# qasimyu/simuscop

Measured on AMD Instinct MI355X. Metric: simulated paired reads/sec (whole node) at 30x WGS PE150, higher is better.
Workload: dtype u32

## Files before the change

simuscop_amd/csrc/sg_kernels.hip:

```cpp
#include <algorithm>
#include <cstdlib>
#include <type_traits>

#include "sg_device.h"

namespace sg {

template <int ROUNDS>
__device__ __forceinline__ void philox4x32(uint32_t c0, uint32_t c1, uint32_t c2, uint32_t c3,
                                           uint32_t k0, uint32_t k1, uint32_t out[4]) {
  const uint32_t M0 = 0xD2511F53u, M1 = 0xCD9E8D57u;
#pragma unroll
  for (int r = 0; r < ROUNDS; r++) {
    const uint64_t p0 = (uint64_t)M0 * c0, p1 = (uint64_t)M1 * c2;
    const uint32_t hi0 = (uint32_t)(p0 >> 32), lo0 = (uint32_t)p0;
    const uint32_t hi1 = (uint32_t)(p1 >> 32), lo1 = (uint32_t)p1;
    c0 = __builtin_amdgcn_bitop3_b32(hi1, c1, k0, 0x96);
    c1 = lo1;
    c2 = __builtin_amdgcn_bitop3_b32(hi0, c3, k1, 0x96);
    c3 = lo0;
    k0 += 0x9E3779B9u;
    k1 += 0xBB67AE85u;
  }
  out[0] = c0; out[1] = c1; out[2] = c2; out[3] = c3;
// ... 22 lines not shown
  philox4x32_10(slot + B.slot_offset, j, f >> 2, dev_ctx(KIND_AUX, mate, B.batch_id), B.k0, B.k1, x);
  uint32_t l = f & 3;
  return l == 0 ? x[0] : l == 1 ? x[1] : l == 2 ? x[2] : x[3];
}

__device__ __forceinline__ uint32_t ndigits(uint32_t v) {
  return v < 10 ? 1 : v < 100 ? 2 : v < 1000 ? 3 : v < 10000 ? 4 : v < 100000 ? 5 : v < 1000000 ? 6
       : v < 10000000 ? 7 : v < 100000000 ? 8 : v < 1000000000 ? 9 : 10;
}

#define PLAN_S 16

__device__ __forceinline__ bool plan_attempt(const DevProfile& P, const DevBatch& B, const sg_window& win, uint64_t w,
                                             uint32_t attempt, uint64_t clen, uint32_t c3, PairRec& r, const uint32_t* isz_row,
                                             uint32_t seg_size, uint64_t chain_off) {
  uint32_t x[4];
  philox4x32_10((uint32_t)w + B.win_offset, attempt, 0, c3, B.k0, B.k1, x);
  const double frac = __dmul_rn((double)x[0], 1.0 / 4294967296.0);
  const double v = __dadd_rn((double)win.spos, __dmul_rn((double)win.len, frac));
  const uint32_t pos = (uint32_t)(long long)v;
  uint32_t isz;
  if (B.paired) isz = isz_row ? (uint32_t)P.isz_min + row_search(isz_row, P.isz_lg, x[1]) : (uint32_t)P.fixed_isz;
  else isz = win.len;
  const uint64_t avail = clen - (win.hap_base + pos);
  const uint32_t flen = avail < (uint64_t)isz ? (uint32_t)avail : isz;
  const uint32_t strand = B.paired ? 0u : (x[2] >> 31);
  r.win = (uint32_t)w; r.fl = flen | (strand << 31);
  r.namepos = pos % seg_size;
  r.foff = chain_off + win.hap_base + pos;
  r.pad = 0;
  return flen >= (uint32_t)P.L;
}

__global__ __launch_bounds__(256) void plan_kernel(DevProfile P, DevBatch B) {
  __shared__ uint32_t isz_lds[1025];
  const uint32_t* isz_row = P.isz_row;
  if (P.isz_row && P.isz_lg <= 10u) {
    for (uint32_t i = threadIdx.x; i < (1u << P.isz_lg) + 1u; i += blockDim.x) isz_lds[i] = P.isz_row[i];
    isz_row = isz_lds;
  }
  __syncthreads();
  if (blockIdx.x == 0)
    for (uint32_t i = threadIdx.x; i < kTotalsBytes / 4u; i += blockDim.x) ((uint32_t*)B.totals)[i] = 0u;
  const uint64_t gid = (uint64_t)blockIdx.x * blockDim.x + threadIdx.x;
  const uint64_t w = gid / PLAN_S;
  const uint32_t j = (uint32_t)(gid % PLAN_S);
  if (w >= B.n_windows) return;
  const sg_window win = B.windows[w];
  const int n = win.n_reads;
  const uint32_t planned = n <= 0 ? 0u : (B.paired ? ((uint32_t)n + 1u) / 2u : (uint32_t)n);
  const uint64_t clen = B.chain_len[win.chain];
  const uint32_t seg_size = B.seg_size[win.seg];
  const uint64_t chain_off = B.chain_off[win.chain];
  const uint32_t c3 = dev_ctx(KIND_PLAN, 0, B.batch_id);
  const uint64_t last_start = win.hap_base + win.spos + win.len - 1u;
  const uint64_t need = B.paired ? (uint64_t)P.isz_hi : (uint64_t)win.len;
  const uint32_t shortest = B.paired ? (uint32_t)P.isz_lo : win.len;
  const bool safe = last_start + need <= clen && shortest >= (uint32_t)P.L;
  if (safe) {
    for (uint32_t k = j; k < planned; k += PLAN_S) {
      PairRec r;
      plan_attempt(P, B, win, w, k, clen, c3, r, isz_row, seg_size, chain_off);
      r.k = k;
      B.pairs[win.slot_base + k] = r;
    }
    if (j == 0) B.win_actual[w] = planned;
    return;
  }
  if (j != 0) return;
  uint32_t done = 0, fail = 0, attempt = 0;
  while (done < planned) {
    PairRec r;
    if (!plan_attempt(P, B, win, w, attempt++, clen, c3, r, isz_row, seg_size, chain_off)) {
      if (++fail > 1000) break;
      continue;
    }
    r.k = done;
    B.pairs[win.slot_base + done] = r;
    done++;
  }
  for (uint32_t k = done; k < planned; k++) {
    PairRec r;
    r.win = (uint32_t)w; r.namepos = 0; r.fl = 0; r.k = k; r.foff = 0; r.pad = 0;
    B.pairs[win.slot_base + k] = r;
  }
  B.win_actual[w] = done;
}

__global__ __launch_bounds__(64) void namebase_kernel(DevBatch B) {
  const uint32_t s = blockIdx.x;
  const uint32_t lane = threadIdx.x;
  const uint32_t w0 = B.seg_first_window[s], w1 = B.seg_first_window[s + 1];
  uint32_t carry = 0;
  for (uint32_t base = w0; base < w1; base += 64) {
    uint32_t w = base + lane;
    uint32_t v = w < w1 ? B.win_actual[w] : 0u;
    uint32_t incl = v;
#pragma unroll
    for (int d = 1; d < 64; d <<= 1) {
      uint32_t t = __shfl_up(incl, d);
      if ((int)lane >= d) incl += t;
    }
    if (w < w1) B.win_namebase[w] = carry + incl - v;
    carry += __shfl(incl, 63);
  }
  if (lane == 0) atomicAdd((unsigned long long*)&B.totals[2], (unsigned long long)carry);
}

__device__ __forceinline__ void wave_lds_sync() {
  __builtin_amdgcn_fence(__ATOMIC_RELEASE, "wavefront");
  __builtin_amdgcn_wave_barrier();
  __builtin_amdgcn_fence(__ATOMIC_ACQUIRE, "wavefront");
}

__device__ __forceinline__ uint64_t rec_offset(const DevBatch& B, uint32_t m, uint32_t t) {
  const uint32_t blk = t >> 8;
  const uint64_t* segbase = (const uint64_t*)((const uint8_t*)B.totals + kTotalsSegBase);
  return segbase[m * 16u + (blk >> B.seg_shift)] + B.blkbase[(size_t)m * ((B.n_slots + 255u) >> 8) + blk] +
         B.recloc[(size_t)m * B.n_slots + t];
}

__global__ __launch_bounds__(256) void indel_kernel(DevProfile P, DevBatch B) {
  __shared__ uint4 row_lds[256 * 3];
  __shared__ uint16_t cand[512];
  __shared__ uint32_t cand_n;
  __shared__ uint2 found[2][256];
  __shared__ uint32_t found_first[2][256];
  __shared__ uint32_t wave_len[2][4];
  const uint32_t tid = threadIdx.x, lane = tid & 63u, wv = tid >> 6;
  const uint32_t t = blockIdx.x * blockDim.x + tid;
  const uint32_t nm = B.paired ? 2u : 1u;
  uint4* const wave_rows = row_lds + (tid & ~63u) * 3u;
  uint4* const my_row = wave_rows + lane * 3u;
  const uint32_t t_wave = t - lane;
  __shared__ uint64_t gap_lds[256];
  const uint64_t* gap = P.gap_row;
  if ((uint32_t)P.L + 1u <= 256u) {
    for (uint32_t i = tid; i <= (uint32_t)P.L; i += blockDim.x) gap_lds[i] = P.gap_row[i];
    gap = gap_lds;
  }
  if (tid == 0u) cand_n = 0u;
  const bool in_batch = t < B.n_slots;
  PairRec rec = {};
  if (in_batch) rec = B.pairs[t];
  const uint32_t flen = rec.fl & 0x7FFFFFFFu;
  const bool live = flen != 0u;
  const uint32_t L = (uint32_t)P.L;
  uint32_t fragcount = 0, touches_bad[2] = {0, 0};
  const uint64_t foff = rec.foff;
  const uint32_t rev1 = rec.fl >> 31;
  if (live) {
    fragcount = B.win_namebase[rec.win] + rec.k + 1u;
    for (uint32_t m = 0; m < nm; m++) {
      const bool rev = B.paired ? (m == 1u) : (rev1 != 0u);
      const uint64_t t0 = (rev ? foff + flen - L : foff) - 8u, t1 = t0 + L + 24u;
      uint32_t bad = 0;
      for (uint64_t b = t0 >> 6; b <= (t1 >> 6); b++) bad |= (B.chains_bad[b >> 4] >> (b & 15u)) & 1u;
      touches_bad[m] = bad;
    }
  }
  __syncthreads();
  for (uint32_t m = 0; m < nm; m++) {
    found[m][tid] = make_uint2(0u, 0u);
    found_first[m][tid] = 0u;
    bool has = false;
    if (live) {
      uint32_t x4[4];
      philox4x32_10(t + B.slot_offset, 0u, 0, dev_ctx(KIND_INDEL, m, B.batch_id), B.k0, B.k1, x4);
      const uint64_t x = ((uint64_t)x4[1] << 32) | x4[0];
      has = !(x < gap[L]);
    }
    const unsigned long long hm = __ballot(has);
    if (hm) {
      uint32_t base = 0;
      if (lane == (uint32_t)__builtin_ctzll(hm)) base = atomicAdd(&cand_n, (uint32_t)__popcll(hm));
      base = __shfl(base, __builtin_ctzll(hm), 64);
      if (has) cand[base + (uint32_t)__popcll(hm & ((1ull << lane) - 1ull))] = (uint16_t)(tid | (m << 8));
    }
  }
  __syncthreads();
  {
    const uint32_t nc = cand_n;
#pragma unroll 1
    for (uint32_t i = tid; i < nc; i += blockDim.x) {
      const uint32_t e16 = cand[i], lt = e16 & 255u, m = e16 >> 8;
      const uint32_t tt = blockIdx.x * blockDim.x + lt;
      uint32_t* ev = B.events + ((size_t)m * B.n_slots + tt) * SG_MAX_EVENTS;
      const uint32_t c3 = dev_ctx(KIND_INDEL, m, B.batch_id);
      int j = 0, dl = 0;
      uint32_t nev = 0, first_ev = 0, e = 0;
#pragma unroll 1
      while (j < (int)L) {
        uint32_t x4[4];
        philox4x32_10(tt + B.slot_offset, e++, 0, c3, B.k0, B.k1, x4);
        const uint64_t x = ((uint64_t)x4[1] << 32) | x4[0], y = ((uint64_t)x4[3] << 32) | x4[2];
        const int room = (int)L - j;
        if (x < gap[room]) break;
        int lo = 0, hi = room - 1;
        while (lo < hi) {
          const int mid = (lo + hi + 1) >> 1;
          if (x < gap[mid]) lo = mid; else hi = mid - 1;
        }
        const int jj = j + lo;
        const bool is_ins = __umul64hi(y, P.evB) < P.evA;
        j = jj + 1;
        if (is_ins) {
          uint32_t len = row_search(P.ins_row, P.ins_lg, aux_draw(B, tt, (uint32_t)jj, 0, m));
          if (len > 0) {
            if (nev < SG_MAX_EVENTS) ev[nev] = ev_pack((uint32_t)jj, len, 0);
            if (nev == 0) first_ev = ev_pack((uint32_t)jj, len, 0);
            nev++;
            dl += (int)len;
          }
        } else {
          uint32_t len = row_search(P.del_row, P.del_lg, aux_draw(B, tt, (uint32_t)jj, 0, m));
          if (len > 0) {
            uint32_t k = min((uint32_t)((int)L - jj), len);
            if (nev < SG_MAX_EVENTS) ev[nev] = ev_pack((uint32_t)jj, k, 1);
            if (nev == 0) first_ev = ev_pack((uint32_t)jj, k, 1);
            nev++;
            dl -= (int)k;
            j = jj + (int)k;
          }
        }
      }
      found[m][lt] = make_uint2(nev, (uint32_t)dl);
      found_first[m][lt] = first_ev;
    }
  }
  __syncthreads();
  const uint32_t namepos = rec.namepos;
  const uint32_t hdr = B.prefix_len + ndigits(namepos) + 1u + ndigits(fragcount) + (B.paired ? 2u : 0u) + 1u;
  uint32_t mate_at = 0;
  my_row[0] = live ? make_uint4((uint32_t)foff, (uint32_t)(foff >> 32), namepos, fragcount) : make_uint4(0, 0, 0, 0);
  my_row[2] = make_uint4(0, 0, 0, 0);
  if (live && hdr - B.prefix_len <= 16u) {
    uint8_t* hb = (uint8_t*)(my_row + 2);
    uint32_t o = 0;
    auto put_dec = [&](uint32_t v) {
      const uint32_t nd = ndigits(v);
      for (uint32_t k = nd; k-- > 0u;) {
        const uint32_t qd = v / 10u;
        hb[o + k] = (uint8_t)('0' + (v - qd * 10u));
        v = qd;
      }
      o += nd;
    };
    put_dec(namepos);
    hb[o++] = '#';
    put_dec(fragcount);
    if (B.paired) { hb[o++] = '/'; mate_at = o; hb[o++] = '1'; }
    hb[o] = '\n';
  }
  uint32_t rl[2] = {0, 0};
  for (uint32_t m = 0; m < nm; m++) {
    if (m == 1u) {
      wave_lds_sync();
      if (mate_at) ((uint8_t*)(my_row + 2))[mate_at] = '2';
    }
    uint4 mid = make_uint4(0, 0, 0, 0);
    if (live) {
      const uint2 f = found[m][tid];
      uint32_t nev = f.x;
      int dl = (int)f.y;
      if ((int)L + dl < 50) { nev = 0; dl = 0; }
      if (nev > SG_MAX_EVENTS) { atomicOr((unsigned long long*)&B.totals[3], 1ull); nev = 0; dl = 0; }
      const uint32_t np = (uint32_t)((int)L + dl);
      rl[m] = hdr + 2u * np + 4u;
      const uint32_t rev = B.paired ? m : rev1;
      mid = make_uint4(flen | (touches_bad[m] << 30) | (rev << 31), np | (nev << 16) | (hdr << 22), 0xFFFFFFFFu / np + 1u,
                       nev == 1u ? found_first[m][tid] : 0u);
    }
    my_row[1] = mid;
    if (t_wave < B.n_slots) {
      wave_lds_sync();
      uint4* dst = B.meta + ((size_t)m * B.n_slots + t_wave) * 3;
      const uint32_t n_pieces = min(B.n_slots - t_wave, 64u) * 3u;
#pragma unroll
      for (uint32_t i = 0; i < 3u; i++) {
        const uint32_t q = i * 64u + lane;
        if (q < n_pieces) dst[q] = wave_rows[q];
      }
    }
  }
  uint32_t incl[2];
  for (uint32_t m = 0; m < nm; m++) {
    uint32_t v = rl[m];
#pragma unroll
    for (int d = 1; d < 64; d <<= 1) {
      const uint32_t up = __shfl_up(v, d, 64);
      if ((int)lane >= d) v += up;
    }
    incl[m] = v;
    if (lane == 63u) wave_len[m][wv] = v;
  }
  __syncthreads();
  for (uint32_t m = 0; m < nm; m++) {
    uint32_t base = 0, all = 0;
#pragma unroll
    for (uint32_t i = 0; i < 4u; i++) {
      const uint32_t w = wave_len[m][i];
      if (i < wv) base += w;
      all += w;
    }
// ... 1553 lines not shown
}
__global__ __launch_bounds__(256) void planned_kernel(const sg_window* __restrict__ rows, uint64_t n, int32_t paired, uint32_t* __restrict__ planned) {
  const uint64_t w = (uint64_t)blockIdx.x * blockDim.x + threadIdx.x;
  if (w >= n) return;
  const int32_t r = rows[w].n_reads;
  planned[w] = r <= 0 ? 0u : (paired ? ((uint32_t)r + 1u) / 2u : (uint32_t)r);
}
__global__ __launch_bounds__(256) void slot_base_kernel(sg_window* __restrict__ rows, uint64_t n, const uint64_t* __restrict__ off) {
  const uint64_t w = (uint64_t)blockIdx.x * blockDim.x + threadIdx.x;
  if (w < n) rows[w].slot_base = (uint32_t)off[w];
}
__global__ __launch_bounds__(64) void seg_slots_kernel(const uint64_t* __restrict__ off, const uint32_t* __restrict__ seg_first, uint32_t n_act,
                                                       const uint64_t* __restrict__ total, uint64_t* __restrict__ out) {
  const uint32_t a = blockIdx.x * blockDim.x + threadIdx.x;
  if (a < n_act) out[a] = off[seg_first[a]];
  if (a == n_act) out[a] = *total;
}
__global__ __launch_bounds__(256) void slice_kernel(const sg_window* __restrict__ all, uint64_t w_lo, uint64_t n, uint32_t a0, uint32_t slot_lo,
                                                    sg_window* __restrict__ out) {
  const uint64_t w = (uint64_t)blockIdx.x * blockDim.x + threadIdx.x;
  if (w >= n) return;
  sg_window o = all[w_lo + w];
  o.seg -= a0;
  o.slot_base -= slot_lo;
  out[w] = o;
}

__global__ void mail_kernel(const uint64_t* __restrict__ totals, uint64_t* __restrict__ mail) {
  if (threadIdx.x < 5u) mail[threadIdx.x] = totals[threadIdx.x];
}
void launch_mail(const uint64_t* totals, uint64_t* mail, hipStream_t s) {
  hipLaunchKernelGGL(mail_kernel, dim3(1), dim3(64), 0, s, totals, mail);
}
void launch_plan(const DevProfile& P, const DevBatch& B, hipStream_t s) {
  if (!B.n_windows) return;
  uint32_t grid = (uint32_t)((B.n_windows * PLAN_S + 255) / 256);
  hipLaunchKernelGGL(plan_kernel, dim3(grid), dim3(256), 0, s, P, B);
}
void launch_namebase(const DevBatch& B, hipStream_t s) {
  if (!B.n_segs) return;
  hipLaunchKernelGGL(namebase_kernel, dim3(B.n_segs), dim3(64), 0, s, B);
}
void launch_indel(const DevProfile& P, const DevBatch& B, hipStream_t s) {
  if (!B.n_slots) return;
  hipLaunchKernelGGL(indel_kernel, dim3((B.n_slots + 255) / 256), dim3(256), 0, s, P, B);
}
void launch_header(const DevProfile& P, const DevBatch& B, hipStream_t s) {
  if (!B.n_slots) return;
  const bool fast = emit_uses_fast_kernel(P, B);
  if (fast && B.prefix_len <= 16u) return;
  dim3 grid((B.n_slots + 255) / 256, B.paired ? 2 : 1);
  hipLaunchKernelGGL(header_kernel, grid, dim3(256), 0, s, B);
}
uint32_t scan_blocks(uint32_t n) { return (n + SCAN_TILE - 1) / SCAN_TILE; }
uint32_t record_seg_shift(uint32_t n_slots) {
  const uint32_t nblk = (n_slots + 255u) >> 8;
  uint32_t k = 0;
  while (((nblk + (1u << k) - 1u) >> k) > 16u) k++;
  return k;
}
void launch_scan(const DevBatch& B, hipStream_t s) {
  if (!B.n_slots) return;
  hipLaunchKernelGGL(block_base_kernel, dim3(16, B.paired ? 2 : 1), dim3(1024), 0, s, B);
}
void launch_scan_u32(const uint32_t* in, uint32_t n, uint64_t* bsum, uint64_t* out, uint64_t* total, hipStream_t s) {
  if (!n) return;
  const uint32_t nblk = scan_blocks(n);
  hipLaunchKernelGGL(scan_reduce_kernel, dim3(nblk, 1), dim3(SCAN_BLOCK), 0, s, in, n, bsum, nblk);
  hipLaunchKernelGGL(scan_sums_kernel, dim3(1), dim3(1024), 0, s, bsum, nblk, total);
  hipLaunchKernelGGL(scan_apply_kernel, dim3(nblk, 1), dim3(SCAN_BLOCK), 0, s, in, n, bsum, nblk, out);
}
static const size_t kLdsBytes = 160 * 1024;
template <int KT, bool SL>
static void launch_emit_variant(const DevProfile& P, const DevBatch& B, dim3 grid, size_t lds, uint32_t sub_rows, uint32_t TI,
// ... 151 lines not shown
```

simuscop_amd/csrc/sg_api.cpp:

```cpp
#include <hip/hip_runtime.h>

#include <algorithm>
#include <chrono>
#include <cstdio>
#include <cstdlib>
#include <cstring>
#include <map>
#include <mutex>
#include <string>
#include <vector>

#include "sg_api.h"
#include "sg_deflate.h"
#include "sg_tables.h"
#include "sg_truth.h"

namespace {

struct BlockCache {
  struct Block { void* p; size_t cap; int dev; };
  std::mutex mu;
  std::vector<Block> blocks;
  size_t held = 0;
  static size_t limit() {
// ... 140 lines not shown
  p = nullptr; cap = 0;
}

struct sg_outputs {
  int device = 0;
  hipStream_t stream = nullptr;
  DevBuf text[2], gz[2];
  uint64_t text_bytes[2] = {0, 0}, gz_bytes[2] = {0, 0};
  std::string err;
  ~sg_outputs() {
    if (stream) { (void)hipStreamSynchronize(stream); (void)hipStreamDestroy(stream); }
  }
};

sg_ctx::~sg_ctx() {
  (void)hipSetDevice(device);
  if (stream) (void)hipStreamSynchronize(stream);
  for (sg_outputs* o : spare) delete o;
  if (evs_created)
    for (auto& ev : evs) (void)hipEventDestroy(ev);
  if (own_stream) { (void)hipStreamSynchronize(own_stream); (void)hipStreamDestroy(own_stream); }
  if (mail) (void)hipHostFree(mail);
}

static int finish_plan(sg_ctx* ctx, uint64_t nw, uint32_t n_segs, uint32_t n_slots, uint32_t batch_id, uint32_t first_window,
                       uint32_t first_slot, int32_t paired, const char* name_prefix) {
  const size_t plen = name_prefix ? strlen(name_prefix) : 0;
  const uint32_t nm = paired ? 2 : 1;
  SG_ENSURE(ctx->prefix, plen + 16);
  SG_ENSURE(ctx->pairs, ((size_t)n_slots + 1) * sizeof(sg::PairRec));
  SG_ENSURE(ctx->win_actual, (nw + 1) * 4);
  SG_ENSURE(ctx->win_namebase, (nw + 1) * 4);
  SG_ENSURE(ctx->events, ((size_t)nm * n_slots + 1) * 4 * SG_MAX_EVENTS);
  SG_ENSURE(ctx->recoff, ((size_t)nm * n_slots + 1) * 4);
  SG_ENSURE(ctx->meta, ((size_t)nm * n_slots + 1) * 48);
  SG_ENSURE(ctx->totals, sg::kTotalsBytes);
  SG_ENSURE(ctx->bsum, ((size_t)nm * ((n_slots + 255) / 256) + 1) * 8);
  SG_HIP(hipMemcpyAsync(ctx->prefix.p, name_prefix, plen, hipMemcpyHostToDevice, ctx->stream));
  SG_HIP(hipStreamSynchronize(ctx->stream));

  sg::DevBatch& B = ctx->B;
  B.windows = ctx->windows.as<sg_window>();
  B.n_windows = nw;
  B.seg_size = ctx->segmeta.as<uint32_t>();
  B.seg_first_window = ctx->segmeta.as<uint32_t>() + n_segs;
  B.n_segs = n_segs;
  B.n_slots = n_slots;
  B.batch_id = batch_id;
  B.win_offset = first_window;
  B.slot_offset = first_slot;
  B.paired = paired ? 1 : 0;
  B.prefix = ctx->prefix.as<uint8_t>();
  B.prefix_len = (uint32_t)plen;
  for (int i = 0; i < 4; i++) B.prefix_w[i] = 0;
  for (size_t i = 0; i < plen && i < 16; i++) B.prefix_w[i / 4] |= (uint32_t)(uint8_t)name_prefix[i] << (8 * (i % 4));
  B.pairs = ctx->pairs.as<sg::PairRec>();
  B.win_actual = ctx->win_actual.as<uint32_t>();
  B.win_namebase = ctx->win_namebase.as<uint32_t>();
  B.events = ctx->events.as<uint32_t>();
  B.recloc = ctx->recoff.as<uint32_t>();
  B.blkbase = ctx->bsum.as<uint64_t>();
  B.seg_shift = sg::record_seg_shift((uint32_t)n_slots);
  B.meta = ctx->meta.as<uint4>();
  B.totals = ctx->totals.as<uint64_t>();
  B.slowq_count = (uint32_t*)(B.totals + 4);
  ctx->have_plan = true;
  ctx->sampled = false;
  ctx->results_valid = false;
  return SG_OK;
}

static int pack_chains(sg_ctx* ctx, size_t total) {
  const size_t q = total / 4, badb = total / 64 / 8;
  SG_ENSURE(ctx->chains2, 2 * q + badb + 64);
  uint8_t* p = ctx->chains2.as<uint8_t>();
  sg::launch_pack2(ctx->chains.as<uint8_t>(), total, (uint32_t*)p, (uint32_t*)(p + q), (uint16_t*)(p + 2 * q), ctx->stream);
  ctx->B.chains2_fwd = p;
  ctx->B.chains2_rc = p + q;
  ctx->B.chains_bad = (const uint16_t*)(p + 2 * q);
  ctx->B.chains_total = total;
  return SG_OK;
}

static sg_ctx::ChainLayout chain_layout(int32_t n_chains, const uint64_t* lens) {
  const size_t PAD = 256;
  sg_ctx::ChainLayout L;
  L.len.assign(lens, lens + n_chains);
  L.total = PAD;
  for (int c = 0; c < n_chains; c++) {
    L.off.push_back(L.total);
    L.total += (lens[c] + PAD + 63) & ~(size_t)63;
  }
// ... 1026 lines not shown
  hipStream_t s = ctx->stream;
  B.out[0] = ctx->out1.as<uint8_t>();
  B.out[1] = ctx->out2.as<uint8_t>();
  B.out_cap[0] = ctx->out1.cap;
  B.out_cap[1] = ctx->out2.cap;
  B.slowq = nullptr;
  B.slowq_cap = 0;
  if (sg::emit_uses_fast_kernel(ctx->P, B)) {
    uint64_t cap = std::max<uint64_t>(1u << 16, 2ull * B.n_slots);
    if (const char* e = getenv("SG_SLOWQ_CAP")) cap = std::max<uint64_t>(1, strtoull(e, nullptr, 10));
    cap = std::min<uint64_t>(cap, 1ull << 30);
    SG_ENSURE(ctx->slowq, cap * 8 * (B.paired ? 2 : 1));
    B.slowq = ctx->slowq.as<uint2>();
    B.slowq_cap = (uint32_t)cap;
  }
  if (prof) SG_HIP(hipEventRecord(ctx->evs[5], s));
  sg::launch_header(ctx->P, B, s);
  ctx->emit_path = sg::emit_path(ctx->P, B, false);
  sg::launch_emit(ctx->P, B, s, false, prof ? ctx->evs[7] : nullptr);
  if (prof) SG_HIP(hipEventRecord(ctx->evs[6], s));
  return SG_OK;
}

static int run_pass(sg_ctx* ctx) {
  sg::DevBatch& B = ctx->B;
  B.k0 = (uint32_t)ctx->seed;
  B.k1 = (uint32_t)(ctx->seed >> 32);
  { const char* dg = getenv("SG_DIAG"); B.diag = dg ? (uint32_t)atoi(dg) : 0u; }
  if (const char* fd = getenv("SG_FDIAG")) B.diag = (uint32_t)atoi(fd);
  hipStream_t s = ctx->stream;
  const bool prof = ctx->profiling;
  if (!B.n_windows) SG_HIP(hipMemsetAsync(B.totals, 0, sg::kTotalsBytes, s));
  if (prof) SG_HIP(hipEventRecord(ctx->evs[0], s));
  sg::launch_plan(ctx->P, B, s);
  if (prof) SG_HIP(hipEventRecord(ctx->evs[1], s));
  sg::launch_namebase(B, s);
  if (prof) SG_HIP(hipEventRecord(ctx->evs[2], s));
  sg::launch_indel(ctx->P, B, s);
  if (prof) SG_HIP(hipEventRecord(ctx->evs[3], s));
  sg::launch_scan(B, s);
  if (prof) SG_HIP(hipEventRecord(ctx->evs[4], s));
  SG_HIP(hipGetLastError());
  if (!ctx->out1.p && !ctx->out2.p && !ctx->gz1.p && !ctx->gz2.p && !ctx->spare.empty()) {
    sg_outputs* o = ctx->spare.back();
    std::swap(ctx->out1, o->text[0]); std::swap(ctx->out2, o->text[1]);
    std::swap(ctx->gz1, o->gz[0]); std::swap(ctx->gz2, o->gz[1]);
  }
  ctx->speculative = ctx->out1.p != nullptr && (!B.paired || ctx->out2.p != nullptr) && getenv("SG_NO_SPECULATION") == nullptr;
  if (!ctx->speculative) {
    sg::launch_mail(B.totals, ctx->mail, s);
    SG_HIP(hipStreamSynchronize(s));
    memcpy(ctx->host_totals, ctx->mail, 4 * 8);
    if (ctx->host_totals[3] & 1) return ctx->fail(SG_ERR_OVERFLOW, "sg_sample: a read drew more than SG_MAX_EVENTS sequencing indels");
    SG_ENSURE(ctx->out1, ctx->host_totals[0] + 64);
    if (B.paired) SG_ENSURE(ctx->out2, ctx->host_totals[1] + 64);
  }
  if (int rc = launch_text(ctx, prof)) return rc;
  sg::launch_mail(B.totals, ctx->mail, s);
  SG_HIP(hipGetLastError());
  ctx->sampled = true;
  ctx->pass_pending = true;
  ctx->results_valid = false;
  ctx->gz_valid = false;
  return SG_OK;
}

static int finish_pass(sg_ctx* ctx) {
// ... 354 lines not shown
```

simuscop_amd/csrc/sg_api.h:

```cpp
#pragma once
#include <hip/hip_runtime.h>

#include <map>
#include <string>
#include <utility>
#include <vector>

#include "sg_device.h"
#include "sg_haplotypes.h"

struct DevBuf {
  void* p = nullptr;
  size_t cap = 0;
  int dev = 0;
  DevBuf() = default;
  DevBuf(DevBuf&& o) noexcept : p(std::exchange(o.p, nullptr)), cap(std::exchange(o.cap, 0)), dev(o.dev) {}
  DevBuf& operator=(DevBuf&& o) noexcept {
    if (this != &o) { release(); p = std::exchange(o.p, nullptr); cap = std::exchange(o.cap, 0); dev = o.dev; }
    return *this;
  }
  DevBuf(const DevBuf&) = delete;
  DevBuf& operator=(const DevBuf&) = delete;
  ~DevBuf() { release(); }
  int ensure(size_t bytes);
  void release();
  template <class T> T* as() const { return (T*)p; }
};

extern thread_local std::string g_create_error;

struct sg_outputs;
struct sg_train_session;

struct sg_ctx {
  int device = 0;
  hipStream_t own_stream = nullptr;
  hipStream_t stream = nullptr;
  uint64_t seed = 0;
  std::string err;

  bool have_profile = false, have_haps = false, have_plan = false, sampled = false;
  sg::DevProfile P{};
  sg::DevBatch B{};
  DevBuf tab, chains, chains2, chain_meta, windows, segmeta, prefix, pairs, win_actual, win_namebase, events, recoff, meta, totals, bsum,
      out1, out2, gcw, gco, gcm, slowq, ref_raw, ref_codes, ref_meta, hap_work, gz1, gz2, gz_work,
      infl_src, infl_meta, infl_out, infl_crc,
      defl_src, defl_out;
  struct ChainLayout {
    std::vector<uint64_t> off, len;
    size_t total = 0;
  } hap;
  uint64_t gz_bytes[2] = {0, 0};
  bool gz_valid = false;
  struct Truth {
    uint64_t n_given = 0;
    bool from_build = false, mapped = false, valid = false;
    std::vector<sg_truth_piece> sorted;
    std::vector<uint64_t> chain_first;
    uint64_t rec_bytes = 0, gz_bytes = 0, records = 0, unmapped = 0;
  } truth;
  DevBuf truth_map, truth_work, truth_rec, truth_gz, truth_rows;
  struct Depth {
    bool on = false;
    std::vector<uint64_t> len, off;
    uint64_t slots = 0, m_bases = 0, scanned_starts = 0;
    int64_t scanned = -1;
  } depth;
  DevBuf depth_diff, depth_meta, depth_work, depth_out;
  std::vector<sg_outputs*> spare;
  std::map<uint32_t, DevBuf> wstore;
  std::map<uint32_t, uint64_t> wstore_n;
  DevBuf wplan, wwork;
  struct PlanInfo {
    bool valid = false;
    uint64_t n_windows = 0;
    uint32_t n_active = 0, batch_id = 0;
    int32_t paired = 0;
// ... 41 lines not shown
```

simuscop_amd/csrc/sg_device.h:

```cpp
#pragma once
#include <hip/hip_runtime.h>
#include <stdint.h>

#include "../../include/simuscop_amd.h"

namespace sg {

constexpr size_t kTotalsSegBase = 128 + 2 * 2 * 8 * 128;
constexpr size_t kTotalsBytes = kTotalsSegBase + 2 * 16 * 8 + 64;

constexpr int kBaseRounds = 7;

enum : uint32_t { KIND_HAP = 1, KIND_GC = 2, KIND_PLAN = 3, KIND_INDEL = 4, KIND_AUX = 5, KIND_BASE = 6 };

struct PairRec {
  uint32_t win;
  uint32_t namepos;
  uint32_t fl;
  uint32_t k;
  uint64_t foff;
  uint64_t pad;
};

__host__ __device__ inline uint32_t ev_pack(uint32_t j, uint32_t len, uint32_t del) { return j | (len << 16) | (del << 31); }
// ... 19 lines not shown
  uint32_t remap_packed;
  uint32_t bases_packed;
  uint32_t kmer_off[8];
  uint32_t inv_remap_packed;
};

struct DevBatch {
  const uint8_t* chains;
  const uint64_t* chain_off;
  const uint64_t* chain_len;
  const uint8_t* chains2_fwd;
  const uint8_t* chains2_rc;
  const uint16_t* chains_bad;
  uint64_t chains_total;
  const sg_window* windows;
  uint64_t n_windows;
  const uint32_t* seg_size;
  const uint32_t* seg_first_window;
  uint32_t n_segs;
  uint32_t n_slots;
  uint32_t batch_id;
  uint32_t win_offset, slot_offset;
  int32_t paired;
  const uint8_t* prefix;
  uint32_t prefix_len;
  uint32_t prefix_w[4];
  uint32_t k0, k1;
  uint32_t diag;
  uint32_t strict_bases;
  PairRec* pairs;
  uint32_t* win_actual;
  uint32_t* win_namebase;
  uint32_t* events;
  uint32_t* recloc;
  uint64_t* blkbase;
  uint32_t seg_shift;
  uint4* meta;
  uint64_t* totals;
  uint2* slowq;
  uint32_t* slowq_count;
  uint32_t slowq_cap;
  uint8_t* out[2];
  uint64_t out_cap[2];
};

void launch_plan(const DevProfile& P, const DevBatch& B, hipStream_t s);
void launch_namebase(const DevBatch& B, hipStream_t s);
void launch_indel(const DevProfile& P, const DevBatch& B, hipStream_t s);
void launch_scan(const DevBatch& B, hipStream_t s);
void launch_mail(const uint64_t* totals, uint64_t* mail, hipStream_t s);
void launch_header(const DevProfile& P, const DevBatch& B, hipStream_t s);
void launch_emit(const DevProfile& P, const DevBatch& B, hipStream_t s, bool force_generic, hipEvent_t after_main);
bool emit_uses_fast_kernel(const DevProfile& P, const DevBatch& B);
int emit_variant(const DevProfile& P);
struct EmitPath { int main_kernel; int slow_rows_lds; uint32_t lds_bytes, clean_cap; };
EmitPath emit_path(const DevProfile& P, const DevBatch& B, bool force_generic);
uint32_t record_seg_shift(uint32_t n_slots);
uint32_t scan_blocks(uint32_t n);
void launch_scan_u32(const uint32_t* in, uint32_t n, uint64_t* bsum, uint64_t* out, uint64_t* total, hipStream_t s);
void launch_encode(uint8_t* buf, size_t bytes, hipStream_t s);
void launch_gc(const uint8_t* chains, const uint64_t* chain_off, const sg_gc_window* wins, uint64_t n, int32_t* out, hipStream_t s);
void launch_tile(const sg_window_gen* gens, const uint64_t* prefix, uint32_t n_gens, uint64_t n, uint32_t frag, const uint64_t* seg_first,
                 sg_gc_window* out, uint32_t* seg_ord, uint32_t* win_ord, hipStream_t s);
void launch_seg_sum(const double* wt, const uint64_t* seg_first, uint32_t n_segs, double* out, hipStream_t s);
void launch_window_reads(const sg_window_gen* gens, const uint64_t* prefix, uint32_t n_gens, uint64_t n, uint32_t frag, const double* wt,
                         const sg_active_seg* act, const uint32_t* seg_first, uint32_t n_act, sg_window* rows, unsigned long long* seg_sum,
                         int32_t paired, uint32_t* planned, hipStream_t s);
void launch_slot_base(sg_window* rows, uint64_t n, const uint64_t* off, const uint32_t* seg_first, uint32_t n_act, const uint64_t* total,
                      uint64_t* seg_slots, hipStream_t s);
void launch_slice(const sg_window* all, uint64_t w_lo, uint64_t n, uint32_t a0, uint32_t slot_lo, sg_window* out, hipStream_t s);
void launch_gc_weight(const int32_t* gc, const sg_gc_window* wins, const uint32_t* seg_ord, const uint32_t* win_ord, uint64_t n,
                      const double* means, double std, const double* Q, uint32_t lg_cells, uint32_t frag, int32_t full_tile_form,
                      uint32_t ctx24, uint64_t seed, double* out, hipStream_t s);

}
```

Baseline: 2.152 billion.

## Widen namebase scan to multi-wave blocks and stage indel length tables in LDS

The namebase scan kernel now runs one block of up to 1024 threads per segment instead of a single wave, using a double-buffered LDS table of per-wave sums so long segments are scanned in fewer serial iterations. In the indel kernel, the insertion and deletion length tables are copied into the reused row_lds buffer when they fit, and the walk loop is templated so row_search reads from LDS instead of global memory. Global loads for the gap row and length tables are issued early and written to LDS after the pair record is read, so their latency overlaps other loads. The chains_bad check is replaced with two-word loads and a bitmask when the span fits, instead of a per-bit loop. The cost is more LDS aliasing of row_lds and an extra __syncthreads per namebase iteration.

```diff
diff --git a/simuscop_amd/csrc/sg_kernels.hip b/simuscop_amd/csrc/sg_kernels.hip
--- a/simuscop_amd/csrc/sg_kernels.hip
+++ b/simuscop_amd/csrc/sg_kernels.hip
@@ -133,13 +133,16 @@
   B.win_actual[w] = done;
 }
 
-__global__ __launch_bounds__(64) void namebase_kernel(DevBatch B) {
+#define NAMEBASE_MAX_THREADS 1024
+
+__global__ __launch_bounds__(NAMEBASE_MAX_THREADS) void namebase_kernel(DevBatch B) {
+  __shared__ uint32_t wave_sum[2][NAMEBASE_MAX_THREADS / 64];
   const uint32_t s = blockIdx.x;
-  const uint32_t lane = threadIdx.x;
+  const uint32_t tid = threadIdx.x, lane = tid & 63u, wv = tid >> 6, n_waves = blockDim.x >> 6;
   const uint32_t w0 = B.seg_first_window[s], w1 = B.seg_first_window[s + 1];
-  uint32_t carry = 0;
-  for (uint32_t base = w0; base < w1; base += 64) {
-    uint32_t w = base + lane;
+  uint32_t carry = 0, par = 0;
+  for (uint32_t base = w0; base < w1; base += blockDim.x, par ^= 1u) {
+    uint32_t w = base + tid;
     uint32_t v = w < w1 ? B.win_actual[w] : 0u;
     uint32_t incl = v;
 #pragma unroll
@@ -147,10 +150,18 @@
       uint32_t t = __shfl_up(incl, d);
       if ((int)lane >= d) incl += t;
     }
-    if (w < w1) B.win_namebase[w] = carry + incl - v;
-    carry += __shfl(incl, 63);
-  }
-  if (lane == 0) atomicAdd((unsigned long long*)&B.totals[2], (unsigned long long)carry);
+    if (lane == 63u) wave_sum[par][wv] = incl;
+    __syncthreads();
+    uint32_t before = 0, all = 0;
+    for (uint32_t i = 0; i < n_waves; i++) {
+      const uint32_t x = wave_sum[par][i];
+      if (i < wv) before += x;
+      all += x;
+    }
+    if (w < w1) B.win_namebase[w] = carry + before + incl - v;
+    carry += all;
+  }
+  if (tid == 0) atomicAdd((unsigned long long*)&B.totals[2], (unsigned long long)carry);
 }
 
 __device__ __forceinline__ void wave_lds_sync() {
@@ -179,32 +190,67 @@
   uint4* const wave_rows = row_lds + (tid & ~63u) * 3u;
   uint4* const my_row = wave_rows + lane * 3u;
   const uint32_t t_wave = t - lane;
-  __shared__ uint64_t gap_lds[256];
-  const uint64_t* gap = P.gap_row;
-  if ((uint32_t)P.L + 1u <= 256u) {
-    for (uint32_t i = tid; i <= (uint32_t)P.L; i += blockDim.x) gap_lds[i] = P.gap_row[i];
-    gap = gap_lds;
-  }
-  if (tid == 0u) cand_n = 0u;
   const bool in_batch = t < B.n_slots;
   PairRec rec = {};
   if (in_batch) rec = B.pairs[t];
+  const uint32_t L = (uint32_t)P.L;
+  __shared__ uint64_t gap_lds[256];
+  const uint64_t* gap = P.gap_row;
+  const bool stage_gap = L + 1u <= 256u;
+  uint64_t gap_w = 0;
+  if (stage_gap && tid <= L) gap_w = P.gap_row[tid];
+  uint32_t* const len_lds = (uint32_t*)row_lds;
+  const uint32_t n_ins = (1u << P.ins_lg) + 1u, n_del = (1u << P.del_lg) + 1u;
+  const bool stage_len = P.ins_lg < 16u && P.del_lg < 16u && n_ins + n_del <= (uint32_t)(sizeof(row_lds) / 4u);
+  const uint32_t n_len = stage_len ? n_ins + n_del : 0u;
+  auto len_word = [&](uint32_t i) { return i < n_ins ? P.ins_row[i] : P.del_row[i - n_ins]; };
+  uint32_t len_w = 0;
+  if (tid < n_len) len_w = len_word(tid);
+  if (tid == 0u) cand_n = 0u;
   const uint32_t flen = rec.fl & 0x7FFFFFFFu;
   const bool live = flen != 0u;
-  const uint32_t L = (uint32_t)P.L;
   uint32_t fragcount = 0, touches_bad[2] = {0, 0};
   const uint64_t foff = rec.foff;
   const uint32_t rev1 = rec.fl >> 31;
+  const bool two_words = (L + 24u) / 64u + 2u <= 16u;
+  uint64_t blk0[2] = {0, 0}, blk1[2] = {0, 0};
+  for (uint32_t m = 0; m < 2u; m++) {
+    const bool rev = B.paired ? (m == 1u) : (rev1 != 0u);
+    const uint64_t t0 = (rev ? foff + flen - L : foff) - 8u, t1 = t0 + L + 24u;
+    blk0[m] = t0 >> 6;
+    blk1[m] = t1 >> 6;
+  }
   if (live) {
-    fragcount = B.win_namebase[rec.win] + rec.k + 1u;
-    for (uint32_t m = 0; m < nm; m++) {
-      const bool rev = B.paired ? (m == 1u) : (rev1 != 0u);
-      const uint64_t t0 = (rev ? foff + flen - L : foff) - 8u, t1 = t0 + L + 24u;
-      uint32_t bad = 0;
-      for (uint64_t b = t0 >> 6; b <= (t1 >> 6); b++) bad |= (B.chains_bad[b >> 4] >> (b & 15u)) & 1u;
-      touches_bad[m] = bad;
-    }
-  }
+    const uint32_t namebase = B.win_namebase[rec.win];
+    if (two_words) {
+      uint32_t lo[2] = {0, 0}, hi[2] = {0, 0};
+#pragma unroll
+      for (uint32_t m = 0; m < 2u; m++)
+        if (m < nm) {
+          lo[m] = B.chains_bad[blk0[m] >> 4];
+          hi[m] = B.chains_bad[(blk0[m] >> 4) + 1u];
+        }
+#pragma unroll
+      for (uint32_t m = 0; m < 2u; m++) {
+        const uint32_t n_blk = (uint32_t)(blk1[m] - blk0[m]) + 1u;
+        const uint32_t mask = ((1u << n_blk) - 1u) << (uint32_t)(blk0[m] & 15u);
+        touches_bad[m] = ((lo[m] | (hi[m] << 16)) & mask) != 0u ? 1u : 0u;
+      }
+    } else {
+      for (uint32_t m = 0; m < nm; m++) {
+        uint32_t bad = 0;
+        for (uint64_t b = blk0[m]; b <= blk1[m]; b++) bad |= (B.chains_bad[b >> 4] >> (b & 15u)) & 1u;
+        touches_bad[m] = bad;
+      }
+    }
+    fragcount = namebase + rec.k + 1u;
+  }
+  if (stage_gap) {
+    if (tid <= L) gap_lds[tid] = gap_w;
+    gap = gap_lds;
+  }
+  if (tid < n_len) len_lds[tid] = len_w;
+  for (uint32_t i = tid + 256u; i < n_len; i += 256u) len_lds[i] = len_word(i);
   __syncthreads();
   for (uint32_t m = 0; m < nm; m++) {
     found[m][tid] = make_uint2(0u, 0u);
@@ -225,7 +271,9 @@
     }
   }
   __syncthreads();
-  {
+  auto walk = [&](auto in_lds) {
+    const uint32_t* const ins_row = decltype(in_lds)::value ? len_lds : P.ins_row;
+    const uint32_t* const del_row = decltype(in_lds)::value ? len_lds + n_ins : P.del_row;
     const uint32_t nc = cand_n;
 #pragma unroll 1
     for (uint32_t i = tid; i < nc; i += blockDim.x) {
@@ -251,7 +299,7 @@
         const bool is_ins = __umul64hi(y, P.evB) < P.evA;
         j = jj + 1;
         if (is_ins) {
-          uint32_t len = row_search(P.ins_row, P.ins_lg, aux_draw(B, tt, (uint32_t)jj, 0, m));
+          uint32_t len = row_search(ins_row, P.ins_lg, aux_draw(B, tt, (uint32_t)jj, 0, m));
           if (len > 0) {
             if (nev < SG_MAX_EVENTS) ev[nev] = ev_pack((uint32_t)jj, len, 0);
             if (nev == 0) first_ev = ev_pack((uint32_t)jj, len, 0);
@@ -259,7 +307,7 @@
             dl += (int)len;
           }
         } else {
-          uint32_t len = row_search(P.del_row, P.del_lg, aux_draw(B, tt, (uint32_t)jj, 0, m));
+          uint32_t len = row_search(del_row, P.del_lg, aux_draw(B, tt, (uint32_t)jj, 0, m));
           if (len > 0) {
             uint32_t k = min((uint32_t)((int)L - jj), len);
             if (nev < SG_MAX_EVENTS) ev[nev] = ev_pack((uint32_t)jj, k, 1);
@@ -273,7 +321,9 @@
       found[m][lt] = make_uint2(nev, (uint32_t)dl);
       found_first[m][lt] = first_ev;
     }
-  }
+  };
+  if (stage_len) walk(std::true_type{});
+  else walk(std::false_type{});
   __syncthreads();
   const uint32_t namepos = rec.namepos;
   const uint32_t hdr = B.prefix_len + ndigits(namepos) + 1u + ndigits(fragcount) + (B.paired ? 2u : 0u) + 1u;
@@ -1942,7 +1992,10 @@
 }
 void launch_namebase(const DevBatch& B, hipStream_t s) {
   if (!B.n_segs) return;
-  hipLaunchKernelGGL(namebase_kernel, dim3(B.n_segs), dim3(64), 0, s, B);
+  const uint64_t per_seg = (B.n_windows + B.n_segs - 1) / B.n_segs;
+  uint32_t threads = 64;
+  while (threads < NAMEBASE_MAX_THREADS && threads < per_seg) threads <<= 1;
+  hipLaunchKernelGGL(namebase_kernel, dim3(B.n_segs), dim3(threads), 0, s, B);
 }
 void launch_indel(const DevProfile& P, const DevBatch& B, hipStream_t s) {
   if (!B.n_slots) return;
```

Result: faster. 2.181 billion, median of 6 (+1.4%).

## Move indel walk out of indel kernel into a fused plan+walk front kernel

Applied to the files above, without the earlier changes.

The indel event walk, which depends only on slot index and RNG and not on the plan output, moves out of indel_kernel into a new front_kernel. That kernel interleaves plan blocks and walk blocks in one launch. Walk results are packed into a new 64-bit per-slot walk buffer that indel_kernel reads back. The walk compacts candidates per wave instead of per block, removing block-wide barriers and a shared atomic, and caches the gap, insertion and deletion tables in LDS when they fit. This trades an extra global buffer write and read and a larger LDS footprint for overlapping the walk with planning and lighter synchronisation. The walk now runs for every slot in the batch rather than only live ones, so it may do extra work on empty slots.

```diff
diff --git a/simuscop_amd/csrc/sg_api.cpp b/simuscop_amd/csrc/sg_api.cpp
--- a/simuscop_amd/csrc/sg_api.cpp
+++ b/simuscop_amd/csrc/sg_api.cpp
@@ -196,6 +196,7 @@
   SG_ENSURE(ctx->win_actual, (nw + 1) * 4);
   SG_ENSURE(ctx->win_namebase, (nw + 1) * 4);
   SG_ENSURE(ctx->events, ((size_t)nm * n_slots + 1) * 4 * SG_MAX_EVENTS);
+  SG_ENSURE(ctx->walk, ((size_t)nm * n_slots + 1) * 8);
   SG_ENSURE(ctx->recoff, ((size_t)nm * n_slots + 1) * 4);
   SG_ENSURE(ctx->meta, ((size_t)nm * n_slots + 1) * 48);
   SG_ENSURE(ctx->totals, sg::kTotalsBytes);
@@ -222,6 +223,7 @@
   B.win_actual = ctx->win_actual.as<uint32_t>();
   B.win_namebase = ctx->win_namebase.as<uint32_t>();
   B.events = ctx->events.as<uint32_t>();
+  B.walk = ctx->walk.as<uint64_t>();
   B.recloc = ctx->recoff.as<uint32_t>();
   B.blkbase = ctx->bsum.as<uint64_t>();
   B.seg_shift = sg::record_seg_shift((uint32_t)n_slots);
@@ -1314,7 +1316,7 @@
   const bool prof = ctx->profiling;
   if (!B.n_windows) SG_HIP(hipMemsetAsync(B.totals, 0, sg::kTotalsBytes, s));
   if (prof) SG_HIP(hipEventRecord(ctx->evs[0], s));
-  sg::launch_plan(ctx->P, B, s);
+  sg::launch_front(ctx->P, B, s);
   if (prof) SG_HIP(hipEventRecord(ctx->evs[1], s));
   sg::launch_namebase(B, s);
   if (prof) SG_HIP(hipEventRecord(ctx->evs[2], s));
diff --git a/simuscop_amd/csrc/sg_api.h b/simuscop_amd/csrc/sg_api.h
--- a/simuscop_amd/csrc/sg_api.h
+++ b/simuscop_amd/csrc/sg_api.h
@@ -42,7 +42,7 @@
   bool have_profile = false, have_haps = false, have_plan = false, sampled = false;
   sg::DevProfile P{};
   sg::DevBatch B{};
-  DevBuf tab, chains, chains2, chain_meta, windows, segmeta, prefix, pairs, win_actual, win_namebase, events, recoff, meta, totals, bsum,
+  DevBuf tab, chains, chains2, chain_meta, windows, segmeta, prefix, pairs, win_actual, win_namebase, events, walk, recoff, meta, totals, bsum,
       out1, out2, gcw, gco, gcm, slowq, ref_raw, ref_codes, ref_meta, hap_work, gz1, gz2, gz_work,
       infl_src, infl_meta, infl_out, infl_crc,
       defl_src, defl_out;
diff --git a/simuscop_amd/csrc/sg_device.h b/simuscop_amd/csrc/sg_device.h
--- a/simuscop_amd/csrc/sg_device.h
+++ b/simuscop_amd/csrc/sg_device.h
@@ -75,6 +75,7 @@
   uint32_t* win_actual;
   uint32_t* win_namebase;
   uint32_t* events;
+  uint64_t* walk;
   uint32_t* recloc;
   uint64_t* blkbase;
   uint32_t seg_shift;
@@ -87,7 +88,7 @@
   uint64_t out_cap[2];
 };
 
-void launch_plan(const DevProfile& P, const DevBatch& B, hipStream_t s);
+void launch_front(const DevProfile& P, const DevBatch& B, hipStream_t s);
 void launch_namebase(const DevBatch& B, hipStream_t s);
 void launch_indel(const DevProfile& P, const DevBatch& B, hipStream_t s);
 void launch_scan(const DevBatch& B, hipStream_t s);
diff --git a/simuscop_amd/csrc/sg_kernels.hip b/simuscop_amd/csrc/sg_kernels.hip
--- a/simuscop_amd/csrc/sg_kernels.hip
+++ b/simuscop_amd/csrc/sg_kernels.hip
@@ -78,17 +78,16 @@
   return flen >= (uint32_t)P.L;
 }
 
-__global__ __launch_bounds__(256) void plan_kernel(DevProfile P, DevBatch B) {
-  __shared__ uint32_t isz_lds[1025];
+__device__ __forceinline__ void plan_block(const DevProfile& P, const DevBatch& B, uint32_t* isz_lds, uint32_t blk) {
   const uint32_t* isz_row = P.isz_row;
   if (P.isz_row && P.isz_lg <= 10u) {
     for (uint32_t i = threadIdx.x; i < (1u << P.isz_lg) + 1u; i += blockDim.x) isz_lds[i] = P.isz_row[i];
     isz_row = isz_lds;
   }
   __syncthreads();
-  if (blockIdx.x == 0)
+  if (blk == 0)
     for (uint32_t i = threadIdx.x; i < kTotalsBytes / 4u; i += blockDim.x) ((uint32_t*)B.totals)[i] = 0u;
-  const uint64_t gid = (uint64_t)blockIdx.x * blockDim.x + threadIdx.x;
+  const uint64_t gid = (uint64_t)blk * blockDim.x + threadIdx.x;
   const uint64_t w = gid / PLAN_S;
   const uint32_t j = (uint32_t)(gid % PLAN_S);
   if (w >= B.n_windows) return;
@@ -166,12 +165,125 @@
          B.recloc[(size_t)m * B.n_slots + t];
 }
 
+constexpr uint32_t kWalkRowLg = 8;
+
+struct WalkLds {
+  uint64_t gap[256];
+  uint64_t found[4][128];
+  uint32_t ins[(1u << kWalkRowLg) + 1u], del[(1u << kWalkRowLg) + 1u];
+  uint8_t cand[4][128];
+};
+union FrontLds {
+  uint32_t isz[1025];
+  WalkLds walk;
+};
+
+__device__ __forceinline__ uint64_t walk_pack(uint32_t nev, int dl, uint32_t first_ev, uint32_t L) {
+  const uint32_t n16 = min(nev, 0xFFFFu);
+  const uint32_t d16 = (uint32_t)min(dl, 65535 - (int)L) & 0xFFFFu;
+  return (uint64_t)(n16 | (d16 << 16)) | ((uint64_t)first_ev << 32);
+}
+__device__ __forceinline__ int walk_dl(uint32_t lo_word, uint32_t L) {
+  const int d = (int)lo_word >> 16;
+  return d < -(int)L ? d + 65536 : d;
+}
+
+template <bool LDS_TABLES>
+__device__ __forceinline__ void walk_block(const DevProfile& P, const DevBatch& B, WalkLds& S, uint32_t blk) {
+  const uint32_t tid = threadIdx.x, lane = tid & 63u, wv = tid >> 6;
+  const uint32_t t = blk * blockDim.x + tid;
+  const uint32_t nm = B.paired ? 2u : 1u;
+  const uint32_t L = (uint32_t)P.L;
+  if (LDS_TABLES) {
+    for (uint32_t i = tid; i <= L; i += blockDim.x) S.gap[i] = P.gap_row[i];
+    for (uint32_t i = tid; i < (1u << P.ins_lg) + 1u; i += blockDim.x) S.ins[i] = P.ins_row[i];
+    for (uint32_t i = tid; i < (1u << P.del_lg) + 1u; i += blockDim.x) S.del[i] = P.del_row[i];
+    __syncthreads();
+  }
+  auto gap_at = [&](uint32_t k) -> uint64_t { return LDS_TABLES ? S.gap[k] : P.gap_row[k]; };
+  const bool in_batch = t < B.n_slots;
+  uint64_t* const wfound = S.found[wv];
+  uint8_t* const wcand = S.cand[wv];
+  uint32_t nc = 0;
+  for (uint32_t m = 0; m < nm; m++) {
+    wfound[m * 64u + lane] = 0ull;
+    bool has = false;
+    if (in_batch) {
+      uint32_t x4[4];
+      philox4x32_10(t + B.slot_offset, 0u, 0, dev_ctx(KIND_INDEL, m, B.batch_id), B.k0, B.k1, x4);
+      const uint64_t x = ((uint64_t)x4[1] << 32) | x4[0];
+      has = !(x < gap_at(L));
+    }
+    const unsigned long long hm = __ballot(has);
+    if (has) wcand[nc + (uint32_t)__popcll(hm & ((1ull << lane) - 1ull))] = (uint8_t)(lane | (m << 6));
+    nc += (uint32_t)__popcll(hm);
+  }
+  wave_lds_sync();
+#pragma unroll 1
+  for (uint32_t i = lane; i < nc; i += 64u) {
+    const uint32_t e8 = wcand[i], lt = e8 & 63u, m = e8 >> 6;
+    const uint32_t tt = t - lane + lt;
+    uint32_t* ev = B.events + ((size_t)m * B.n_slots + tt) * SG_MAX_EVENTS;
+    const uint32_t c3 = dev_ctx(KIND_INDEL, m, B.batch_id);
+    int j = 0, dl = 0;
+    uint32_t nev = 0, first_ev = 0, e = 0;
+#pragma unroll 1
+    while (j < (int)L) {
+      uint32_t x4[4];
+      philox4x32_10(tt + B.slot_offset, e++, 0, c3, B.k0, B.k1, x4);
+      const uint64_t x = ((uint64_t)x4[1] << 32) | x4[0], y = ((uint64_t)x4[3] << 32) | x4[2];
+      const int room = (int)L - j;
+      if (x < gap_at((uint32_t)room)) break;
+      int lo = 0, hi = room - 1;
+      while (lo < hi) {
+        const int mid = (lo + hi + 1) >> 1;
+        if (x < gap_at((uint32_t)mid)) lo = mid; else hi = mid - 1;
+      }
+      const int jj = j + lo;
+      const bool is_ins = __umul64hi(y, P.evB) < P.evA;
+      j = jj + 1;
+      const uint32_t a = aux_draw(B, tt, (uint32_t)jj, 0, m);
+      if (is_ins) {
+        const uint32_t len = LDS_TABLES ? row_search(S.ins, P.ins_lg, a) : row_search(P.ins_row, P.ins_lg, a);
+        if (len > 0) {
+          if (nev < SG_MAX_EVENTS) ev[nev] = ev_pack((uint32_t)jj, len, 0);
+          if (nev == 0) first_ev = ev_pack((uint32_t)jj, len, 0);
+          nev++;
+          dl += (int)len;
+        }
+      } else {
+        const uint32_t len = LDS_TABLES ? row_search(S.del, P.del_lg, a) : row_search(P.del_row, P.del_lg, a);
+        if (len > 0) {
+          uint32_t k = min((uint32_t)((int)L - jj), len);
+          if (nev < SG_MAX_EVENTS) ev[nev] = ev_pack((uint32_t)jj, k, 1);
+          if (nev == 0) first_ev = ev_pack((uint32_t)jj, k, 1);
+          nev++;
+          dl -= (int)k;
+          j = jj + (int)k;
+        }
+      }
+    }
+    wfound[m * 64u + lt] = walk_pack(nev, dl, first_ev, L);
+  }
+  wave_lds_sync();
+  if (in_batch)
+    for (uint32_t m = 0; m < nm; m++) B.walk[(size_t)m * B.n_slots + t] = wfound[m * 64u + lane];
+}
+
+__global__ __launch_bounds__(256) void front_kernel(DevProfile P, DevBatch B, uint32_t n_plan, uint32_t n_walk) {
+  __shared__ FrontLds S;
+  const uint64_t n = (uint64_t)n_plan + n_walk, b = blockIdx.x;
+  const uint32_t w0 = (uint32_t)(b * n_walk / n), w1 = (uint32_t)((b + 1u) * n_walk / n);
+  if (w1 == w0) {
+    plan_block(P, B, S.isz, (uint32_t)b - w0);
+    return;
+  }
+  if ((uint32_t)P.L + 1u <= 256u && P.ins_lg <= kWalkRowLg && P.del_lg <= kWalkRowLg) walk_block<true>(P, B, S.walk, w0);
+  else walk_block<false>(P, B, S.walk, w0);
+}
+
 __global__ __launch_bounds__(256) void indel_kernel(DevProfile P, DevBatch B) {
   __shared__ uint4 row_lds[256 * 3];
-  __shared__ uint16_t cand[512];
-  __shared__ uint32_t cand_n;
-  __shared__ uint2 found[2][256];
-  __shared__ uint32_t found_first[2][256];
   __shared__ uint32_t wave_len[2][4];
   const uint32_t tid = threadIdx.x, lane = tid & 63u, wv = tid >> 6;
   const uint32_t t = blockIdx.x * blockDim.x + tid;
@@ -179,23 +291,21 @@
   uint4* const wave_rows = row_lds + (tid & ~63u) * 3u;
   uint4* const my_row = wave_rows + lane * 3u;
   const uint32_t t_wave = t - lane;
-  __shared__ uint64_t gap_lds[256];
-  const uint64_t* gap = P.gap_row;
-  if ((uint32_t)P.L + 1u <= 256u) {
-    for (uint32_t i = tid; i <= (uint32_t)P.L; i += blockDim.x) gap_lds[i] = P.gap_row[i];
-    gap = gap_lds;
-  }
-  if (tid == 0u) cand_n = 0u;
   const bool in_batch = t < B.n_slots;
   PairRec rec = {};
   if (in_batch) rec = B.pairs[t];
   const uint32_t flen = rec.fl & 0x7FFFFFFFu;
   const bool live = flen != 0u;
   const uint32_t L = (uint32_t)P.L;
+  uint2 found[2] = {make_uint2(0u, 0u), make_uint2(0u, 0u)};
   uint32_t fragcount = 0, touches_bad[2] = {0, 0};
   const uint64_t foff = rec.foff;
   const uint32_t rev1 = rec.fl >> 31;
   if (live) {
+    for (uint32_t m = 0; m < nm; m++) {
+      const uint64_t f = B.walk[(size_t)m * B.n_slots + t];
+      found[m] = make_uint2((uint32_t)f, (uint32_t)(f >> 32));
+    }
     fragcount = B.win_namebase[rec.win] + rec.k + 1u;
     for (uint32_t m = 0; m < nm; m++) {
       const bool rev = B.paired ? (m == 1u) : (rev1 != 0u);
@@ -205,76 +315,6 @@
       touches_bad[m] = bad;
     }
   }
-  __syncthreads();
-  for (uint32_t m = 0; m < nm; m++) {
-    found[m][tid] = make_uint2(0u, 0u);
-    found_first[m][tid] = 0u;
-    bool has = false;
-    if (live) {
-      uint32_t x4[4];
-      philox4x32_10(t + B.slot_offset, 0u, 0, dev_ctx(KIND_INDEL, m, B.batch_id), B.k0, B.k1, x4);
-      const uint64_t x = ((uint64_t)x4[1] << 32) | x4[0];
-      has = !(x < gap[L]);
-    }
-    const unsigned long long hm = __ballot(has);
-    if (hm) {
-      uint32_t base = 0;
-      if (lane == (uint32_t)__builtin_ctzll(hm)) base = atomicAdd(&cand_n, (uint32_t)__popcll(hm));
-      base = __shfl(base, __builtin_ctzll(hm), 64);
-      if (has) cand[base + (uint32_t)__popcll(hm & ((1ull << lane) - 1ull))] = (uint16_t)(tid | (m << 8));
-    }
-  }
-  __syncthreads();
-  {
-    const uint32_t nc = cand_n;
-#pragma unroll 1
-    for (uint32_t i = tid; i < nc; i += blockDim.x) {
-      const uint32_t e16 = cand[i], lt = e16 & 255u, m = e16 >> 8;
-      const uint32_t tt = blockIdx.x * blockDim.x + lt;
-      uint32_t* ev = B.events + ((size_t)m * B.n_slots + tt) * SG_MAX_EVENTS;
-      const uint32_t c3 = dev_ctx(KIND_INDEL, m, B.batch_id);
-      int j = 0, dl = 0;
-      uint32_t nev = 0, first_ev = 0, e = 0;
-#pragma unroll 1
-      while (j < (int)L) {
-        uint32_t x4[4];
-        philox4x32_10(tt + B.slot_offset, e++, 0, c3, B.k0, B.k1, x4);
-        const uint64_t x = ((uint64_t)x4[1] << 32) | x4[0], y = ((uint64_t)x4[3] << 32) | x4[2];
-        const int room = (int)L - j;
-        if (x < gap[room]) break;
-        int lo = 0, hi = room - 1;
-        while (lo < hi) {
-          const int mid = (lo + hi + 1) >> 1;
-          if (x < gap[mid]) lo = mid; else hi = mid - 1;
-        }
-        const int jj = j + lo;
-        const bool is_ins = __umul64hi(y, P.evB) < P.evA;
-        j = jj + 1;
-        if (is_ins) {
-          uint32_t len = row_search(P.ins_row, P.ins_lg, aux_draw(B, tt, (uint32_t)jj, 0, m));
-          if (len > 0) {
-            if (nev < SG_MAX_EVENTS) ev[nev] = ev_pack((uint32_t)jj, len, 0);
-            if (nev == 0) first_ev = ev_pack((uint32_t)jj, len, 0);
-            nev++;
-            dl += (int)len;
-          }
-        } else {
-          uint32_t len = row_search(P.del_row, P.del_lg, aux_draw(B, tt, (uint32_t)jj, 0, m));
-          if (len > 0) {
-            uint32_t k = min((uint32_t)((int)L - jj), len);
-            if (nev < SG_MAX_EVENTS) ev[nev] = ev_pack((uint32_t)jj, k, 1);
-            if (nev == 0) first_ev = ev_pack((uint32_t)jj, k, 1);
-            nev++;
-            dl -= (int)k;
-            j = jj + (int)k;
-          }
-        }
-      }
-      found[m][lt] = make_uint2(nev, (uint32_t)dl);
-      found_first[m][lt] = first_ev;
-    }
-  }
-  __syncthreads();
   const uint32_t namepos = rec.namepos;
   const uint32_t hdr = B.prefix_len + ndigits(namepos) + 1u + ndigits(fragcount) + (B.paired ? 2u : 0u) + 1u;
   uint32_t mate_at = 0;
@@ -306,16 +346,16 @@
     }
     uint4 mid = make_uint4(0, 0, 0, 0);
     if (live) {
-      const uint2 f = found[m][tid];
-      uint32_t nev = f.x;
-      int dl = (int)f.y;
+      const uint2 f = found[m];
+      uint32_t nev = f.x & 0xFFFFu;
+      int dl = walk_dl(f.x, L);
       if ((int)L + dl < 50) { nev = 0; dl = 0; }
       if (nev > SG_MAX_EVENTS) { atomicOr((unsigned long long*)&B.totals[3], 1ull); nev = 0; dl = 0; }
       const uint32_t np = (uint32_t)((int)L + dl);
       rl[m] = hdr + 2u * np + 4u;
       const uint32_t rev = B.paired ? m : rev1;
       mid = make_uint4(flen | (touches_bad[m] << 30) | (rev << 31), np | (nev << 16) | (hdr << 22), 0xFFFFFFFFu / np + 1u,
-                       nev == 1u ? found_first[m][tid] : 0u);
+                       nev == 1u ? f.y : 0u);
     }
     my_row[1] = mid;
     if (t_wave < B.n_slots) {
@@ -1935,10 +1975,10 @@
 void launch_mail(const uint64_t* totals, uint64_t* mail, hipStream_t s) {
   hipLaunchKernelGGL(mail_kernel, dim3(1), dim3(64), 0, s, totals, mail);
 }
-void launch_plan(const DevProfile& P, const DevBatch& B, hipStream_t s) {
+void launch_front(const DevProfile& P, const DevBatch& B, hipStream_t s) {
   if (!B.n_windows) return;
-  uint32_t grid = (uint32_t)((B.n_windows * PLAN_S + 255) / 256);
-  hipLaunchKernelGGL(plan_kernel, dim3(grid), dim3(256), 0, s, P, B);
+  const uint32_t n_plan = (uint32_t)((B.n_windows * PLAN_S + 255) / 256), n_walk = (B.n_slots + 255u) / 256u;
+  hipLaunchKernelGGL(front_kernel, dim3(n_plan + n_walk), dim3(256), 0, s, P, B, n_plan, n_walk);
 }
 void launch_namebase(const DevBatch& B, hipStream_t s) {
   if (!B.n_segs) return;
```

Result: no change. 2.143 billion before, 2.145 billion after (median of 6 runs) (+0.1%).
